# shaneson0/attacking_federate_learning

Measured on AMD Instinct MI355X. Metric: aggregation rounds/sec at N clients x D params (Bulyan), higher is better.
Workload: dtype f32 (Gram: fp16x2 split of every fp32 operand, 3 fp16 MFMAs per block, fp32/fp64 accumulate; <= 2e-7 of |gi||gj| vs f...

## Files before the change

attacking_federate_learning_amd/csrc/gram_planes.hip:

```cpp
#include "common.hpp"

#include <cstring>
#include <type_traits>

namespace byz {
namespace {

constexpr int kWgRows = 256;
constexpr int kWgCols = 128;
constexpr int kSlab = 128;
constexpr int kThreads = 512;
constexpr int kFragBytes = 1024;
constexpr int kRowBlocks = (kWgRows + kWgCols) / 32;
constexpr int kChunkCols = 8192;
constexpr int kChunkSteps = kChunkCols / 16;
constexpr int kFlushSteps = 16;
constexpr int kSpareRoundsPercent = 10;

typedef float f32x16 __attribute__((ext_vector_type(16)));
typedef float f32x4 __attribute__((ext_vector_type(4)));
typedef __bf16 bf16x8 __attribute__((ext_vector_type(8)));
typedef _Float16 f16x8 __attribute__((ext_vector_type(8)));
typedef uint32_t u32x4 __attribute__((ext_vector_type(4)));

// ... 590 lines not shown

    const int tid = threadIdx.x;
    const int lane = tid & 63;
    const int wave = __builtin_amdgcn_readfirstlane(tid >> 6);
    const unsigned where = static_cast<unsigned>(__builtin_amdgcn_readfirstlane(my_unit->wave[wave].where));
    const int a_slot = static_cast<int>(where & 0xffu);
    const int b_slot = static_cast<int>((where >> 8) & 0xffu);
    unsigned live_blocks = (where >> 16) & 0xffu;
    const int row_in_slab = static_cast<int>((where >> 24) & 1u) * 64;
    const int col_in_slab = static_cast<int>((where >> 25) & 1u) * 64;
    const int sum_slot = __builtin_amdgcn_readfirstlane(my_unit->wave[wave].sum_slot);
    const bool live_wave = live_blocks != 0;

    const int step0 = chunk * kChunkSteps;
    int n_stages = static_cast<int>(n_steps) - step0;
    if (n_stages > kChunkSteps) n_stages = kChunkSteps;
    const int n_super = n_stages / 2;

    int64_t piece_off[kPerWave];
#pragma unroll
    for (int i = 0; i < kPerWave; ++i) {
        const int q = wave + NW * i;
        const int rbl = q / PLANES, piece = q % PLANES;
        const int64_t rb = __builtin_amdgcn_readfirstlane(my_unit->rb[rbl]);
        piece_off[i] = (((rb * n_steps + step0) * PLANES + piece) * 64) * 16;
    }
    const unsigned char* lane_base = reinterpret_cast<const unsigned char*>(planes) + lane * 16;
    auto dma_piece = [&](int s, int i) __attribute__((always_inline)) {
        unsigned char* dst = lds + (s % NBUF) * kStage + wave * kFragBytes;
        __builtin_amdgcn_global_load_lds(
            (const __attribute__((address_space(1))) void*)(lane_base + piece_off[i] + static_cast<int64_t>(s) * (PLANES * kFragBytes)),
            (__attribute__((address_space(3))) void*)(dst + i * NW * kFragBytes), 16, 0, 0);
    };
    auto dma = [&](int s) __attribute__((always_inline)) {
#pragma unroll
        for (int i = 0; i < kPerWave; ++i) dma_piece(s, i);
    };

    f32x4 acc[4][4], acc2[4][4];
#pragma unroll
    for (int m = 0; m < 4; ++m)
#pragma unroll
        for (int n = 0; n < 4; ++n)
#pragma unroll
            for (int e = 0; e < 4; ++e) {
                acc[m][n][e] = 0.0f;
                acc2[m][n][e] = 0.0f;
            }

    const int lane_in_image = (lane & 15) + 32 * ((lane >> 4) & 1);
    const int pair_half = lane >> 5;
    auto frag_at = [&](int sp, int rb32, int h, int p) __attribute__((always_inline)) -> frag_t {
        const unsigned char* at = lds + (2 * (sp % (NBUF / 2)) + pair_half) * kStage + rb32 * kRbBytes + p * kFragBytes +
                                  (lane_in_image + 16 * h) * 16;
        return *reinterpret_cast<const frag_t*>(at);
    };
    struct AFrags { frag_t v[2][4]; };
    struct BFrags { frag_t v[2][2]; };
    auto read_a = [&](int sp, AFrags& a, auto mask_c) __attribute__((always_inline)) {
        constexpr unsigned MASK = decltype(mask_c)::value;
#pragma unroll
        for (int p = 0; p < 2; ++p)
#pragma unroll
            for (int m = 0; m < 4; ++m)
                if (((MASK >> ((m / 2) * 2)) & 3u) != 0) a.v[p][m] = frag_at(sp, a_slot + m / 2, m % 2, p);
    };
    auto read_b = [&](int sp, int half, BFrags& b, auto mask_c) __attribute__((always_inline)) {
        constexpr unsigned MASK = decltype(mask_c)::value;
#pragma unroll
        for (int p = 0; p < 2; ++p)
#pragma unroll
            for (int n = 0; n < 2; ++n) b.v[p][n] = frag_at(sp, b_slot + half, n, p);
        (void)MASK;
    };
    auto multiply_half = [&](const AFrags& a, const BFrags& b, auto half_c, auto mask_c) __attribute__((always_inline)) {
        constexpr unsigned MASK = decltype(mask_c)::value;
        constexpr int HALF = decltype(half_c)::value;
        constexpr int pa[3] = {1, 0, 0};
        constexpr int pb[3] = {0, 1, 0};
#pragma unroll
        for (int t = 0; t < 3; ++t)
#pragma unroll
            for (int m = 0; m < 4; ++m)
#pragma unroll
                for (int n = 0; n < 2; ++n)
                    if (((MASK >> ((m / 2) * 2 + HALF)) & 1u) != 0)
                        acc[m][2 * HALF + n] = __builtin_amdgcn_mfma_f32_16x16x32_f16(a.v[pa[t]][m], b.v[pb[t]][n], acc[m][2 * HALF + n], 0, 0, 0);
    };
    auto flush = [&](int sp) __attribute__((always_inline)) {
        if ((sp + 1) % kSuperFlush == 0) {
#pragma unroll
            for (int m = 0; m < 4; ++m)
#pragma unroll
                for (int n = 0; n < 4; ++n)
#pragma unroll
                    for (int e = 0; e < 4; ++e) {
                        acc2[m][n][e] += acc[m][n][e];
                        acc[m][n][e] = 0.0f;
                    }
        }
    };

    for (int a = 0; a < NBUF && a < n_stages; ++a) dma(a);
    {
        const int issued = n_stages < NBUF ? n_stages : NBUF;
        wait_vmcnt_dyn((issued > 2 ? issued - 2 : 0) * kPerWave);
    }
    asm volatile("s_barrier" ::: "memory");
    auto k_loop = [&](auto mask_c) __attribute__((always_inline)) {
        constexpr unsigned MASK = decltype(mask_c)::value;
        constexpr bool kLive = MASK != 0;
        constexpr std::integral_constant<int, 0> h0{};
        constexpr std::integral_constant<int, 1> h1{};
        AFrags a0, a1;
        BFrags b0, b1;
        if (kLive && n_super > 0) {
            read_a(0, a0, mask_c);
            if ((MASK & 5u) != 0) read_b(0, 0, b0, mask_c);
        }
        auto super = [&](int sp, AFrags& a, AFrags& an) __attribute__((always_inline)) {
            if (kLive) {
                if ((MASK & 10u) != 0) read_b(sp, 1, b1, mask_c);
                if ((MASK & 5u) != 0) multiply_half(a, b0, h0, mask_c);
            }
            {
                const int last = 2 * sp + 5 < n_stages - 1 ? 2 * sp + 5 : n_stages - 1;
                const int ahead = last - (2 * sp + 3);
                if (2 * sp + 7 < n_stages) wait_vmcnt<2 * kPerWave>();
                else wait_vmcnt_dyn((ahead > 0 ? ahead : 0) * kPerWave);
            }
            asm volatile("s_waitcnt lgkmcnt(0)\n\ts_barrier" ::: "memory");
            if (2 * sp + NBUF < n_stages) dma(2 * sp + NBUF);
            if (2 * sp + NBUF + 1 < n_stages) dma(2 * sp + NBUF + 1);
            if (kLive) {
                if (sp + 1 < n_super) {
                    read_a(sp + 1, an, mask_c);
                    if ((MASK & 5u) != 0) read_b(sp + 1, 0, b0, mask_c);
                }
                if ((MASK & 10u) != 0) multiply_half(a, b1, h1, mask_c);
                flush(sp);
            }
        };
        auto super8 = [&](int sp, AFrags& a, AFrags& an, auto pos_c) __attribute__((always_inline)) {
            constexpr int POS = decltype(pos_c)::value;
            constexpr bool FRESH = POS == 0, FLUSHING = POS == 7;
            constexpr int pa[3] = {1, 0, 0};
            constexpr int pb[3] = {0, 1, 0};
            const f32x4 zero4 = {0.0f, 0.0f, 0.0f, 0.0f};
            auto walk_n = [](int k) __attribute__((always_inline)) { return ((k / 2) & 1) ? 1 - k % 2 : k % 2; };
#pragma unroll
            for (int k = 0; k < 8; ++k) {
                const int m = k / 2, n = walk_n(k);
                if (k % 2 == 0) b1.v[k / 4][m % 2] = frag_at(sp, b_slot + 1, m % 2, k / 4);
#pragma unroll
                for (int t = 0; t < 3; ++t) {
                    acc[m][n] = __builtin_amdgcn_mfma_f32_16x16x32_f16(a.v[pa[t]][m], b0.v[pb[t]][n], (FRESH && t == 0) ? zero4 : acc[m][n], 0, 0, 0);
                    __builtin_amdgcn_sched_barrier(0);
                }
            }
            wait_vmcnt<2 * kPerWave>();
            asm volatile("s_waitcnt lgkmcnt(0)\n\ts_barrier" ::: "memory");
#pragma unroll
            for (int k = 0; k < 8; ++k) {
                const int m = k / 2, n = walk_n(k);
                if (k < 6) {
                    dma_piece(2 * sp + NBUF + k / 3, k % 3);
#pragma unroll
                    for (int r = 2 * k; r < 2 * k + 2; ++r) {
                        if (r < 8) an.v[r / 4][r % 4] = frag_at(sp + 1, a_slot + (r % 4) / 2, (r % 4) % 2, r / 4);
                        else b0.v[(r - 8) / 2][(r - 8) % 2] = frag_at(sp + 1, b_slot, (r - 8) % 2, (r - 8) / 2);
                    }
                }
#pragma unroll
                for (int t = 0; t < 3; ++t) {
                    acc[m][2 + n] = __builtin_amdgcn_mfma_f32_16x16x32_f16(a.v[pa[t]][m], b1.v[pb[t]][n], (FRESH && t == 0) ? zero4 : acc[m][2 + n], 0, 0, 0);
                    __builtin_amdgcn_sched_barrier(0);
                }
                if constexpr (FLUSHING) {
#pragma unroll
                    for (int e = 0; e < 4; ++e) acc2[m][k % 2][e] += acc[m][k % 2][e];
                }
            }
            if constexpr (FLUSHING) {
#pragma unroll
                for (int m = 0; m < 4; ++m)
#pragma unroll
                    for (int n = 2; n < 4; ++n)
#pragma unroll
                        for (int e = 0; e < 4; ++e) acc2[m][n][e] += acc[m][n][e];
            }
        };
        int sp = 0;
        if constexpr (MASK == 15u) {
            bool any = false;
            for (; 2 * (sp + 7) + NBUF + 1 < n_stages && sp + 8 < n_super; sp += 8) {
                super8(sp + 0, a0, a1, std::integral_constant<int, 0>{});
                super8(sp + 1, a1, a0, std::integral_constant<int, 1>{});
                super8(sp + 2, a0, a1, std::integral_constant<int, 2>{});
                super8(sp + 3, a1, a0, std::integral_constant<int, 3>{});
                super8(sp + 4, a0, a1, std::integral_constant<int, 4>{});
                super8(sp + 5, a1, a0, std::integral_constant<int, 5>{});
                super8(sp + 6, a0, a1, std::integral_constant<int, 6>{});
                super8(sp + 7, a1, a0, std::integral_constant<int, 7>{});
                any = true;
            }
            if (any) {
#pragma unroll
                for (int m = 0; m < 4; ++m)
#pragma unroll
                    for (int n = 0; n < 4; ++n)
#pragma unroll
                        for (int e = 0; e < 4; ++e) acc[m][n][e] = 0.0f;
            }
        }
        for (; sp + 1 < n_super; sp += 2) {
            super(sp, a0, a1);
            super(sp + 1, a1, a0);
        }
        if (sp < n_super) super(sp, a0, a1);
    };
    switch (live_blocks) {
        case 0u: k_loop(std::integral_constant<unsigned, 0u>{}); break;
        case 1u: k_loop(std::integral_constant<unsigned, 1u>{}); break;
        case 3u: k_loop(std::integral_constant<unsigned, 3u>{}); break;
        case 13u: k_loop(std::integral_constant<unsigned, 13u>{}); break;
        default: live_blocks = 15u; k_loop(std::integral_constant<unsigned, 15u>{}); break;
    }
    auto block_live = [&](int m, int n) __attribute__((always_inline)) { return ((live_blocks >> ((m / 2) * 2 + n / 2)) & 1u) != 0; };

    if constexpr (DEFER) {
        if (live_wave) {
            const bool unflushed = (n_super % kSuperFlush) != 0;
            float* out = chunk_sums + (static_cast<int64_t>(chunk) * n_sum_slots + sum_slot) * (kSlab * kSlab);
            float* rag = ragged_sums + static_cast<int64_t>(sum_slot) * (kSlab * kSlab);
#pragma unroll
            for (int m = 0; m < 4; ++m)
#pragma unroll
                for (int n = 0; n < 4; ++n) {
                    if (!block_live(m, n)) continue;
                    const int j = col_in_slab + 16 * n + (lane & 15);
#pragma unroll
                    for (int e = 0; e < 4; ++e) {
                        const int i = row_in_slab + 16 * m + 4 * (lane >> 4) + e;
                        out[i * kSlab + j] = acc2[m][n][e];
                        if (unflushed) rag[i * kSlab + j] = acc[m][n][e];
                    }
                }
        }
        __syncthreads();
        if (tid == 0) __hip_atomic_fetch_add(done, 1, __ATOMIC_RELAXED, __HIP_MEMORY_SCOPE_AGENT);
        return;
    }
    bool lost = false;
    if (chunk > 0) {
        if (tid == 0) {
            unsigned spins = 0;
            while (__hip_atomic_load(tickets + t_list, __ATOMIC_RELAXED, __HIP_MEMORY_SCOPE_AGENT) != chunk) {
                __builtin_amdgcn_s_sleep(8);
                if (++spins > (1u << 26)) {
                    lost = true;
                    break;
                }
            }
            __builtin_amdgcn_fence(__ATOMIC_ACQUIRE, "agent");
        }
        lost = __syncthreads_or(lost ? 1 : 0) != 0;
    }
    if (lost) {
        if (tid == 0) atomicOr(device_status, kStatusLostTicket);
    } else if (live_wave) {
        const bool slab_live = chunk > 0 || slab_live0 != 0;
        const int slab = __builtin_amdgcn_readfirstlane(my_unit->wave[wave].slab);
        const int ti = slab & 0xffff, tj = slab >> 16;
        double* out = partial + (static_cast<int64_t>(ti) * (ti + 1) / 2 + tj) * (kSlab * kSlab);
        const double* un = unscale + static_cast<int64_t>(chunk) * rows_pad;
#pragma unroll
        for (int m = 0; m < 4; ++m)
#pragma unroll
            for (int n = 0; n < 4; ++n) {
                if (!block_live(m, n)) continue;
                const int j = col_in_slab + 16 * n + (lane & 15);
                const double uj = un[static_cast<int64_t>(tj) * kSlab + j];
#pragma unroll
                for (int e = 0; e < 4; ++e) {
                    const int i = row_in_slab + 16 * m + 4 * (lane >> 4) + e;
                    double v = static_cast<double>(acc2[m][n][e]);
                    v += static_cast<double>(acc[m][n][e]);
                    v *= un[static_cast<int64_t>(ti) * kSlab + i] * uj;
                    if (slab_live) v += out[i * kSlab + j];
                    out[i * kSlab + j] = v;
                }
            }
    }
    asm volatile("s_waitcnt vmcnt(0)" ::: "memory");
    __syncthreads();
    if (tid == 0) {
        __builtin_amdgcn_fence(__ATOMIC_RELEASE, "agent");
        asm volatile("s_waitcnt vmcnt(0)" ::: "memory");
        __hip_atomic_store(tickets + t_list, chunk + 1, __ATOMIC_RELAXED, __HIP_MEMORY_SCOPE_AGENT);
        __hip_atomic_fetch_add(done, 1, __ATOMIC_RELAXED, __HIP_MEMORY_SCOPE_AGENT);
    }
}

constexpr int kReduceRun = 8;
__global__ __launch_bounds__(256) void chunk_reduce_kernel(const float* __restrict__ chunk_sums, const float* __restrict__ ragged_sums,
                                                           int n_sum_slots, int n_chunks, int ragged_chunk,
                                                           const int2* __restrict__ slot_slab, const double* __restrict__ unscale,
                                                           int64_t rows_pad, double* __restrict__ partial, int slab_live0,
                                                           int n_blocks32) {
    typedef double f64x4 __attribute__((ext_vector_type(4)));
    const int slot = blockIdx.x;
    const int2 tt = slot_slab[slot];
    const int ti = tt.x, tj = tt.y;
    if (ti < 0) return;
    double* out = partial + (static_cast<int64_t>(ti) * (ti + 1) / 2 + tj) * (kSlab * kSlab);
    const int64_t slab_stride = static_cast<int64_t>(n_sum_slots) * (kSlab * kSlab);
    const float* in = chunk_sums + static_cast<int64_t>(slot) * (kSlab * kSlab);
    const float* rag = ragged_sums + static_cast<int64_t>(slot) * (kSlab * kSlab);
    const int i = static_cast<int>(blockIdx.y) * 32 + (threadIdx.x >> 3), j = (threadIdx.x & 7) * 4;
    for (int jb = 0; jb < kSlab; jb += 32) {
        const int jj = jb + j;
        if (n_blocks32 >= 0) {
            const int rblk = ti * 4 + (i >> 5), cblk = tj * 4 + (jj >> 5);
            if (!(rblk < n_blocks32 && cblk <= rblk)) continue;
        }
        const int idx = i * kSlab + jj;
        f64x4 v = {0.0, 0.0, 0.0, 0.0};
        bool live = slab_live0 != 0;
        if (live) v = *reinterpret_cast<const f64x4*>(out + idx);
        for (int c0 = 0; c0 < n_chunks; c0 += kReduceRun) {
            f32x4 p[kReduceRun];
            double ui[kReduceRun];
            f64x4 uj[kReduceRun];
#pragma unroll
            for (int k = 0; k < kReduceRun; ++k) {
                const int c = c0 + k < n_chunks ? c0 + k : n_chunks - 1;
                p[k] = *reinterpret_cast<const f32x4*>(in + c * slab_stride + idx);
                const double* un = unscale + static_cast<int64_t>(c) * rows_pad;
                ui[k] = un[static_cast<int64_t>(ti) * kSlab + i];
                uj[k] = *reinterpret_cast<const f64x4*>(un + static_cast<int64_t>(tj) * kSlab + jj);
            }
#pragma unroll
            for (int k = 0; k < kReduceRun; ++k) {
                if (c0 + k >= n_chunks) break;
                f64x4 q = {static_cast<double>(p[k][0]), static_cast<double>(p[k][1]), static_cast<double>(p[k][2]),
                           static_cast<double>(p[k][3])};
                if (c0 + k == ragged_chunk) {
                    const f32x4 r = *reinterpret_cast<const f32x4*>(rag + idx);
                    q[0] += static_cast<double>(r[0]); q[1] += static_cast<double>(r[1]);
                    q[2] += static_cast<double>(r[2]); q[3] += static_cast<double>(r[3]);
                }
#pragma unroll
                for (int e = 0; e < 4; ++e) {
                    q[e] *= ui[k] * uj[k][e];
                    v[e] = live ? q[e] + v[e] : q[e];
                }
                live = true;
            }
        }
        *reinterpret_cast<f64x4*>(out + idx) = v;
    }
}

}

bool gram_planes_enabled() { return env_int("BYZ_GRAM_PLANES", 1) != 0; }

void build_gram_units(int64_t t128, int64_t n_blocks32, bool diagonal_units, int share_count, int share_index,
                      std::vector<GramUnit>& units, std::vector<int32_t>& slot_slab) {
    units.clear();
    slot_slab.clear();
    const int64_t t256 = ceil_div(t128, 2);
    auto live_mask = [&](int64_t ti, int64_t tj, int row64, int col64) -> uint32_t {
        if (!(tj <= ti && ti < t128)) return 0u;
        if (n_blocks32 < 0) return 15u;
        uint32_t mask = 0;
        for (int m = 0; m < 2; ++m)
            for (int n = 0; n < 2; ++n) {
                const int64_t rblk = ti * 4 + row64 * 2 + m, cblk = tj * 4 + col64 * 2 + n;
                if (rblk < n_blocks32 && cblk <= rblk) mask |= 1u << (m * 2 + n);
            }
        return mask;
    };
    auto set_wave = [&](GramUnit& u, int wave, int a_slot, int b_slot, int64_t ti, int64_t tj, int row64, int col64,
                        int64_t sum_slot) {
        const uint32_t mask = live_mask(ti, tj, row64, col64);
        GramUnitWave& w = u.wave[wave];
        w.where = static_cast<uint32_t>(a_slot) | static_cast<uint32_t>(b_slot) << 8 | mask << 16 |
                  static_cast<uint32_t>(row64) << 24 | static_cast<uint32_t>(col64) << 25;
        w.sum_slot = mask != 0 ? static_cast<int32_t>(sum_slot) : 0;
        w.slab = mask != 0 ? static_cast<int32_t>(ti | tj << 16) : 0;
    };
    auto slab_slot = [](int64_t ti, int64_t tj) { return ti * (ti + 1) / 2 + tj; };
    int64_t position = 0;
    auto plain = [&](int64_t bi, int64_t tj, bool d1) {
        if (position++ % share_count != share_index) return;
        const int64_t t_list = static_cast<int64_t>(units.size());
        GramUnit u{};
        for (int s = 0; s < 12; ++s) u.rb[s] = static_cast<int32_t>(s < 8 ? bi * 8 + s : tj * 4 + (s - 8));
        for (int wave = 0; wave < 8; ++wave) {
            const int wr = wave / 2, wc = wave % 2;
            const int64_t ti = 2 * bi + wr / 2;
            set_wave(u, wave, 2 * wr, 8 + 2 * wc, ti, tj, wr % 2, wc, diagonal_units ? slab_slot(ti, tj) : 2 * t_list + wr / 2);
        }
        if (d1) set_wave(u, 1, 4, 4, 2 * bi + 1, 2 * bi + 1, 0, 0, slab_slot(2 * bi + 1, 2 * bi + 1));
        units.push_back(u);
        if (!diagonal_units)
            for (int sel = 0; sel < 2; ++sel) {
                const int64_t ti = 2 * bi + sel;
                const bool live = tj <= ti && ti < t128;
                slot_slab.push_back(static_cast<int32_t>(live ? ti : -1));
                slot_slab.push_back(static_cast<int32_t>(live ? tj : -1));
            }
    };
    auto d2 = [&](int64_t first, int64_t count) {
        static const int partial_wave[3] = {3, 7, 5};
        GramUnit u{};
        for (int s = 0; s < 12; ++s) u.rb[s] = static_cast<int32_t>(first * 8 + 4);
        for (int64_t k = 0; k < count; ++k) {
            const int64_t bi = first + k, t = 2 * bi + 1;
            for (int s = 0; s < 4; ++s) u.rb[4 * k + s] = static_cast<int32_t>(bi * 8 + 4 + s);
            set_wave(u, static_cast<int>(k), static_cast<int>(4 * k + 2), static_cast<int>(4 * k), t, t, 1, 0, slab_slot(t, t));
            set_wave(u, partial_wave[k], static_cast<int>(4 * k + 2), static_cast<int>(4 * k + 2), t, t, 1, 1, slab_slot(t, t));
        }
        units.push_back(u);
    };
    const int64_t full_blocks = t128 / 2;
    for (int64_t b0 = 0; b0 < t256; b0 += 4)
        for (int64_t tj = 0; tj < t128 && tj <= 2 * (b0 + 3) + 1; ++tj)
            for (int64_t bi = b0; bi < b0 + 4 && bi < t256; ++bi) {
                if (tj > 2 * bi + 1) continue;
                if (!diagonal_units) {
                    plain(bi, tj, false);
                } else if (tj == 2 * bi + 1) {
                    if (bi % 3 == 2 || bi == full_blocks - 1) d2(bi - bi % 3, bi % 3 + 1);
                } else {
                    plain(bi, tj, tj == 2 * bi);
                }
            }
    if (diagonal_units)
        for (int64_t ti = 0; ti < t128; ++ti)
            for (int64_t tj = 0; tj <= ti; ++tj) {
                slot_slab.push_back(static_cast<int32_t>(ti));
                slot_slab.push_back(static_cast<int32_t>(tj));
            }
}

int launch_gram_planes(byz_ctx* ctx, const float* G, int64_t n_rows, int64_t n_cols, int64_t ld, const int32_t* row_index,
                       double* slabs, int share_count, int share_index, uint8_t* owned_host, bool f16, hipStream_t stream) {
    const int64_t t128 = ceil_div(n_rows, kSlab);
    const int64_t t256 = ceil_div(t128, 2);
    const int64_t rows_pad = t256 * kWgRows;
    bool defer = f16 && env_int("BYZ_GRAM_DEFER", 1) != 0;
    const int n_blocks32 = env_int("BYZ_GRAM_BLOCK_SKIP", 1) != 0 ? static_cast<int>(ceil_div(n_rows, 32)) : -1;
    auto ensure_list = [&](bool diagonal_units) -> int {
        const int64_t order_key = static_cast<int64_t>((f16 ? 1 : 0) + (diagonal_units ? 2 : 0)) * (1ll << 40) + share_count * 65536 + share_index;
        const int64_t blocks_key = f16 ? n_blocks32 : -2;
        if (ctx->plane_order_T != t128 || ctx->plane_order_share != order_key || ctx->plane_order_blocks != blocks_key) {
            ctx->plane_order_host.clear();
            if (f16) {
                if (t128 > 0x7fff) {
                    set_error("gram: more than 32767 slabs per side");
                    return BYZ_E_UNSUPPORTED;
                }
                std::vector<GramUnit> units;
                std::vector<int32_t> slot_slab;
                build_gram_units(t128, n_blocks32, diagonal_units, share_count, share_index, units, slot_slab);
                ctx->plane_units = static_cast<int64_t>(units.size());
                ctx->plane_sum_slots = static_cast<int64_t>(slot_slab.size() / 2);
                ctx->plane_order_host.resize(units.size() * kGramUnitWords);
                if (!units.empty()) std::memcpy(ctx->plane_order_host.data(), units.data(), units.size() * sizeof(GramUnit));
                ctx->plane_order_host.insert(ctx->plane_order_host.end(), slot_slab.begin(), slot_slab.end());
            } else {
                int64_t position = 0;
                auto push = [&](int64_t bi, int64_t tj) {
                    if (position++ % share_count != share_index) return;
                    ctx->plane_order_host.push_back(static_cast<int32_t>(bi));
                    ctx->plane_order_host.push_back(static_cast<int32_t>(tj));
                };
                const int64_t S = ceil_div(t128, 8);
                for (int64_t I = 0; I < S; ++I)
                    for (int64_t J = 0; J <= I; ++J)
                        for (int64_t bi = I * 4; bi < I * 4 + 4 && bi < t256; ++bi)
                            for (int64_t tj = J * 8; tj < J * 8 + 8 && tj <= 2 * bi + 1 && tj < t128; ++tj) push(bi, tj);
                ctx->plane_units = static_cast<int64_t>(ctx->plane_order_host.size() / 2);
                ctx->plane_sum_slots = 0;
            }
            BYZ_TRY(ctx->plane_order.ensure(ctx->plane_order_host.size() * sizeof(int32_t) + 16));
            BYZ_HIP(hipMemcpyAsync(ctx->plane_order.ptr, ctx->plane_order_host.data(),
                                   ctx->plane_order_host.size() * sizeof(int32_t), hipMemcpyHostToDevice, stream));
            BYZ_HIP(hipStreamSynchronize(stream));
            ctx->plane_order_T = t128;
            ctx->plane_order_share = order_key;
            ctx->plane_order_blocks = blocks_key;
        }
        return BYZ_OK;
    };
    const bool diagonal_units = defer && share_count == 1 && n_blocks32 >= 0;
    BYZ_TRY(ensure_list(diagonal_units));
    int64_t n_tiles = ctx->plane_units;
    int64_t n_sum_slots = ctx->plane_sum_slots;
    const int32_t* slot_slab_host = ctx->plane_order_host.data() + n_tiles * kGramUnitWords;
    if (owned_host != nullptr) {
        if (f16) {
            for (int64_t s = 0; s < n_sum_slots; ++s) {
                const int64_t ti = slot_slab_host[2 * s], tj = slot_slab_host[2 * s + 1];
                if (ti >= 0) owned_host[ti * (ti + 1) / 2 + tj] = 1;
            }
        } else {
            for (int64_t t = 0; t < n_tiles; ++t) {
                const int64_t bi = ctx->plane_order_host[2 * t], tj = ctx->plane_order_host[2 * t + 1];
                for (int64_t ti = 2 * bi; ti < 2 * bi + 2 && ti < t128; ++ti)
                    if (tj <= ti) owned_host[ti * (ti + 1) / 2 + tj] = 1;
            }
        }
    }
    if (n_tiles == 0) return BYZ_OK;

    const int n_planes = f16 ? 2 : 3;
    size_t free_b = 0, total_b = 0;
    BYZ_HIP(hipMemGetInfo(&free_b, &total_b));
    int64_t budget = static_cast<int64_t>(env_int("BYZ_GRAM_PLANE_MB", 16384)) << 20;
    const int64_t have = static_cast<int64_t>(ctx->gram_planes.bytes);
    if (budget > have + static_cast<int64_t>(free_b / 2)) budget = have + static_cast<int64_t>(free_b / 2);
    int64_t chunks_per_sc = budget / (rows_pad * 2 * n_planes * kChunkCols);
    const int64_t chunks_total = ceil_div(n_cols, kChunkCols);
    if (chunks_per_sc > chunks_total) chunks_per_sc = chunks_total;
    if (chunks_per_sc < 1) {
        set_error("gram: no room for one 8192-column chunk of 16-bit planes (%lld rows)", (long long)rows_pad);
        return BYZ_E_HIP;
    }
    const int64_t n_sc = ceil_div(chunks_total, chunks_per_sc);
    chunks_per_sc = ceil_div(chunks_total, n_sc);
    const int64_t sc_cols = chunks_per_sc * kChunkCols;
    BYZ_TRY(ctx->gram_planes.ensure(static_cast<size_t>(rows_pad) * 2 * n_planes * sc_cols));
    double* unscale = nullptr;
    if (f16) {
        BYZ_TRY(ctx->plane_unscale.ensure(static_cast<size_t>(rows_pad) * chunks_per_sc * sizeof(double)));
        unscale = ctx->plane_unscale.as<double>();
    }
    u32x4* planes = ctx->gram_planes.as<u32x4>();
    float* chunk_sums = nullptr;
    float* ragged_sums = nullptr;
    if (defer) {
        const size_t per_chunk = static_cast<size_t>(n_sum_slots) * kSlab * kSlab * sizeof(float);
        const size_t want = per_chunk * static_cast<size_t>(chunks_per_sc + 1);
        size_t free_now = 0, total_now = 0;
        BYZ_HIP(hipMemGetInfo(&free_now, &total_now));
        if (want > ctx->gram_chunk_sums.bytes && want - ctx->gram_chunk_sums.bytes > free_now / 2) defer = false;
        if (!defer && diagonal_units) {
            BYZ_TRY(ensure_list(false));
            n_tiles = ctx->plane_units;
            n_sum_slots = ctx->plane_sum_slots;
        }
    }
    if (defer) {
        const size_t per_chunk = static_cast<size_t>(n_sum_slots) * kSlab * kSlab * sizeof(float);
        BYZ_TRY(ctx->gram_chunk_sums.ensure(per_chunk * static_cast<size_t>(chunks_per_sc + 1)));
        chunk_sums = ctx->gram_chunk_sums.as<float>();
        ragged_sums = chunk_sums + (per_chunk / sizeof(float)) * static_cast<size_t>(chunks_per_sc);
    }
    auto kernel16 = defer ? &gram_planes16_kernel<6, true> : &gram_planes16_kernel<6, false>;
    const void* kernel = f16 ? reinterpret_cast<const void*>(kernel16) : reinterpret_cast<const void*>(&gram_planes_kernel<4>);
    const size_t lds_bytes = static_cast<size_t>(f16 ? 6 : 4) * kRowBlocks * n_planes * kFragBytes;
    BYZ_HIP(allow_dynamic_lds(ctx, kernel, static_cast<int>(lds_bytes)));
    const int round_size = env_int("BYZ_GRAM_ROUND", ctx->num_cus / 8);
    const int run = round_size > 0 ? round_size : ctx->num_cus / 8;
    const int64_t per_xcd = ceil_div(n_tiles, 8);
    for (int64_t sc = 0; sc < n_sc; ++sc) {
        const int64_t k0 = sc * sc_cols;
        const int64_t cols = n_cols - k0 < sc_cols ? n_cols - k0 : sc_cols;
        const int64_t n_steps = ceil_div(cols, 32) * 2;
        const int64_t n_chunks = ceil_div(n_steps, kChunkSteps);
        {
            KernelTimer t(ctx, BYZ_K_PLANE_SPLIT, stream);
            if (f16) {
                const dim3 grid(static_cast<unsigned>(n_chunks), static_cast<unsigned>(rows_pad / 32));
                if (env_int("BYZ_GRAM_SPLIT_TWO_PASS", 0) != 0) {
                    plane_split_f16_kernel<<<grid, 256, 0, stream>>>(G, n_rows, n_cols, ld, row_index, k0, n_steps, planes,
                                                                     unscale, rows_pad, nullptr);
                } else {
                    const int64_t pairs = n_chunks * (rows_pad / 32);
                    BYZ_TRY(ctx->split_redo.ensure(static_cast<size_t>(1 + 2 * pairs) * sizeof(int32_t)));
                    int32_t* redo = ctx->split_redo.as<int32_t>();
                    BYZ_HIP(hipMemsetAsync(redo, 0, sizeof(int32_t), stream));
                    plane_split_f16_stream_kernel<<<grid, 256, 0, stream>>>(G, n_rows, n_cols, ld, row_index, k0, n_steps, planes,
                                                                            unscale, rows_pad, redo);
                    BYZ_TRY(check_launch("plane_split_f16_stream_kernel"));
                    const int64_t fix = pairs < 4096 ? pairs : 4096;
                    plane_split_f16_kernel<<<static_cast<unsigned>(fix), 256, 0, stream>>>(G, n_rows, n_cols, ld, row_index, k0,
                                                                                           n_steps, planes, unscale, rows_pad, redo);
                }
            } else {
                const dim3 grid(static_cast<unsigned>(ceil_div(n_steps, kSplitCols / 16)), static_cast<unsigned>(rows_pad / 32));
                plane_split_bf16_kernel<<<grid, 256, 0, stream>>>(G, n_rows, n_cols, ld, row_index, k0, n_steps, planes);
            }
            BYZ_TRY(check_launch("plane_split_kernel"));
        }
        {
            int64_t rounds_per_xcd = 0;
            if (f16) {
                rounds_per_xcd = ceil_div(ceil_div(n_tiles * n_chunks, run), 8);
                rounds_per_xcd += rounds_per_xcd * kSpareRoundsPercent / 100;
            }
            const int64_t grid = f16 ? 8 * run * rounds_per_xcd : 8 * per_xcd * n_chunks;
            const size_t ticket_ints = static_cast<size_t>(n_tiles + 9 + 8 * rounds_per_xcd);
            BYZ_TRY(ctx->gram_tickets.ensure(ticket_ints * sizeof(int)));
            int* tickets = ctx->gram_tickets.as<int>();
            BYZ_HIP(hipMemsetAsync(tickets, 0, ticket_ints * sizeof(int), stream));
            KernelTimer t(ctx, BYZ_K_GRAM, stream);
            if (grid > 0x7fffffff) {
                set_error("gram: grid too large");
                return BYZ_E_UNSUPPORTED;
            }
            const int slab_live0 = sc > 0 ? 1 : 0;
            if (!f16) {
                gram_planes_kernel<4><<<static_cast<unsigned>(grid), kThreads, lds_bytes, stream>>>(
                    planes, n_steps, slabs, static_cast<int>(n_tiles), ctx->plane_order.as<int2>(), static_cast<int>(n_chunks), tickets,
                    round_size, static_cast<int>(t128), slab_live0, n_blocks32, device_status_word(ctx));
            } else {
                kernel16<<<static_cast<unsigned>(grid), kThreads, lds_bytes, stream>>>(
                    planes, n_steps, unscale, rows_pad, slabs, static_cast<int>(n_tiles), ctx->plane_order.as<GramUnit>(),
                    static_cast<int>(n_chunks), tickets, round_size, run, slab_live0, static_cast<int>(n_sum_slots),
                    device_status_word(ctx), chunk_sums, ragged_sums);
            }
            BYZ_TRY(check_launch("gram_planes_kernel"));
        }
        if (defer) {
            KernelTimer t(ctx, BYZ_K_GRAM_REDUCE, stream);
            const int ragged_chunk = (n_steps % kChunkSteps) % kFlushSteps != 0 ? static_cast<int>(n_chunks) - 1 : -1;
            const int2* slot_slab = reinterpret_cast<const int2*>(ctx->plane_order.as<GramUnit>() + n_tiles);
            chunk_reduce_kernel<<<dim3(static_cast<unsigned>(n_sum_slots), 4), 256, 0, stream>>>(
                chunk_sums, ragged_sums, static_cast<int>(n_sum_slots), static_cast<int>(n_chunks), ragged_chunk, slot_slab,
                unscale, rows_pad, slabs, sc > 0 ? 1 : 0, n_blocks32);
            BYZ_TRY(check_launch("chunk_reduce_kernel"));
        }
    }
    return BYZ_OK;
}

}
```

Baseline: 2.058.

## Skip dead row blocks in plane split and retile chunk reduction

The chunk reduction kernel is remapped so each block covers 16 rows by 128 columns, two rows per thread. Whole blocks now exit early when their 32-row block is dead, instead of looping over column groups. Gram units redirect row-block slots no wave reads to slot 0, so those planes are not loaded. The plane split grid shrinks to the highest row block any unit references, and the unscale buffer is zeroed on growth so unsplit rows hold defined values. This cuts wasted split work and memory traffic, at the cost of more host-side scanning and a more complex slot mapping.

```diff
diff --git a/attacking_federate_learning_amd/csrc/gram_planes.hip b/attacking_federate_learning_amd/csrc/gram_planes.hip
--- a/attacking_federate_learning_amd/csrc/gram_planes.hip
+++ b/attacking_federate_learning_amd/csrc/gram_planes.hip
@@ -917,6 +917,7 @@
 }
 
 constexpr int kReduceRun = 8;
+constexpr int kReduceRows = 16;
 __global__ __launch_bounds__(256) void chunk_reduce_kernel(const float* __restrict__ chunk_sums, const float* __restrict__ ragged_sums,
                                                            int n_sum_slots, int n_chunks, int ragged_chunk,
                                                            const int2* __restrict__ slot_slab, const double* __restrict__ unscale,
@@ -927,53 +928,61 @@
     const int2 tt = slot_slab[slot];
     const int ti = tt.x, tj = tt.y;
     if (ti < 0) return;
+    const int i = static_cast<int>(blockIdx.y) * kReduceRows + (threadIdx.x >> 5), j = (threadIdx.x & 31) * 4;
+    if (n_blocks32 >= 0) {
+        const int rblk = ti * 4 + (i >> 5), cblk = tj * 4 + (j >> 5);
+        if (!(rblk < n_blocks32 && cblk <= rblk)) return;
+    }
     double* out = partial + (static_cast<int64_t>(ti) * (ti + 1) / 2 + tj) * (kSlab * kSlab);
     const int64_t slab_stride = static_cast<int64_t>(n_sum_slots) * (kSlab * kSlab);
     const float* in = chunk_sums + static_cast<int64_t>(slot) * (kSlab * kSlab);
     const float* rag = ragged_sums + static_cast<int64_t>(slot) * (kSlab * kSlab);
-    const int i = static_cast<int>(blockIdx.y) * 32 + (threadIdx.x >> 3), j = (threadIdx.x & 7) * 4;
-    for (int jb = 0; jb < kSlab; jb += 32) {
-        const int jj = jb + j;
-        if (n_blocks32 >= 0) {
-            const int rblk = ti * 4 + (i >> 5), cblk = tj * 4 + (jj >> 5);
-            if (!(rblk < n_blocks32 && cblk <= rblk)) continue;
-        }
-        const int idx = i * kSlab + jj;
-        f64x4 v = {0.0, 0.0, 0.0, 0.0};
-        bool live = slab_live0 != 0;
-        if (live) v = *reinterpret_cast<const f64x4*>(out + idx);
-        for (int c0 = 0; c0 < n_chunks; c0 += kReduceRun) {
-            f32x4 p[kReduceRun];
-            double ui[kReduceRun];
-            f64x4 uj[kReduceRun];
-#pragma unroll
-            for (int k = 0; k < kReduceRun; ++k) {
-                const int c = c0 + k < n_chunks ? c0 + k : n_chunks - 1;
-                p[k] = *reinterpret_cast<const f32x4*>(in + c * slab_stride + idx);
-                const double* un = unscale + static_cast<int64_t>(c) * rows_pad;
-                ui[k] = un[static_cast<int64_t>(ti) * kSlab + i];
-                uj[k] = *reinterpret_cast<const f64x4*>(un + static_cast<int64_t>(tj) * kSlab + jj);
-            }
-#pragma unroll
-            for (int k = 0; k < kReduceRun; ++k) {
-                if (c0 + k >= n_chunks) break;
-                f64x4 q = {static_cast<double>(p[k][0]), static_cast<double>(p[k][1]), static_cast<double>(p[k][2]),
-                           static_cast<double>(p[k][3])};
+    const int idx[2] = {i * kSlab + j, (i + 8) * kSlab + j};
+    const double* un_i = unscale + static_cast<int64_t>(ti) * kSlab + i;
+    const double* un_j = unscale + static_cast<int64_t>(tj) * kSlab + j;
+    f64x4 v[2] = {{0.0, 0.0, 0.0, 0.0}, {0.0, 0.0, 0.0, 0.0}};
+    bool live = slab_live0 != 0;
+    if (live) {
+#pragma unroll
+        for (int r = 0; r < 2; ++r) v[r] = *reinterpret_cast<const f64x4*>(out + idx[r]);
+    }
+    for (int c0 = 0; c0 < n_chunks; c0 += kReduceRun) {
+        f32x4 p[kReduceRun][2];
+        double ui[kReduceRun][2];
+        f64x4 uj[kReduceRun];
+#pragma unroll
+        for (int k = 0; k < kReduceRun; ++k) {
+            const int c = c0 + k < n_chunks ? c0 + k : n_chunks - 1;
+#pragma unroll
+            for (int r = 0; r < 2; ++r) {
+                p[k][r] = *reinterpret_cast<const f32x4*>(in + c * slab_stride + idx[r]);
+                ui[k][r] = un_i[static_cast<int64_t>(c) * rows_pad + 8 * r];
+            }
+            uj[k] = *reinterpret_cast<const f64x4*>(un_j + static_cast<int64_t>(c) * rows_pad);
+        }
+#pragma unroll
+        for (int k = 0; k < kReduceRun; ++k) {
+            if (c0 + k >= n_chunks) break;
+#pragma unroll
+            for (int r = 0; r < 2; ++r) {
+                f64x4 q = {static_cast<double>(p[k][r][0]), static_cast<double>(p[k][r][1]), static_cast<double>(p[k][r][2]),
+                           static_cast<double>(p[k][r][3])};
                 if (c0 + k == ragged_chunk) {
-                    const f32x4 r = *reinterpret_cast<const f32x4*>(rag + idx);
-                    q[0] += static_cast<double>(r[0]); q[1] += static_cast<double>(r[1]);
-                    q[2] += static_cast<double>(r[2]); q[3] += static_cast<double>(r[3]);
+                    const f32x4 t = *reinterpret_cast<const f32x4*>(rag + idx[r]);
+                    q[0] += static_cast<double>(t[0]); q[1] += static_cast<double>(t[1]);
+                    q[2] += static_cast<double>(t[2]); q[3] += static_cast<double>(t[3]);
                 }
 #pragma unroll
                 for (int e = 0; e < 4; ++e) {
-                    q[e] *= ui[k] * uj[k][e];
-                    v[e] = live ? q[e] + v[e] : q[e];
-                }
-                live = true;
-            }
-        }
-        *reinterpret_cast<f64x4*>(out + idx) = v;
-    }
+                    q[e] *= ui[k][r] * uj[k][e];
+                    v[r][e] = live ? q[e] + v[r][e] : q[e];
+                }
+            }
+            live = true;
+        }
+    }
+#pragma unroll
+    for (int r = 0; r < 2; ++r) *reinterpret_cast<f64x4*>(out + idx[r]) = v[r];
 }
 
 }
@@ -1006,18 +1015,33 @@
         w.slab = mask != 0 ? static_cast<int32_t>(ti | tj << 16) : 0;
     };
     auto slab_slot = [](int64_t ti, int64_t tj) { return ti * (ti + 1) / 2 + tj; };
+    auto retire_dead_slots = [](GramUnit& u) {
+        uint32_t read = 0;
+        for (int wave = 0; wave < 8; ++wave) {
+            const uint32_t where = u.wave[wave].where;
+            const uint32_t a_slot = where & 0xffu, b_slot = (where >> 8) & 0xffu, mask = (where >> 16) & 0xffu;
+            for (int k = 0; k < 2; ++k) {
+                if (((mask >> (2 * k)) & 3u) != 0) read |= 1u << (a_slot + k);
+                if (((mask >> k) & 5u) != 0) read |= 1u << (b_slot + k);
+            }
+        }
+        for (int s = 1; s < 12; ++s)
+            if (((read >> s) & 1u) == 0) u.rb[s] = u.rb[0];
+    };
     int64_t position = 0;
     auto plain = [&](int64_t bi, int64_t tj, bool d1) {
         if (position++ % share_count != share_index) return;
         const int64_t t_list = static_cast<int64_t>(units.size());
         GramUnit u{};
         for (int s = 0; s < 12; ++s) u.rb[s] = static_cast<int32_t>(s < 8 ? bi * 8 + s : tj * 4 + (s - 8));
+        const int b_base = tj == 2 * bi ? 0 : tj == 2 * bi + 1 ? 4 : 8;
         for (int wave = 0; wave < 8; ++wave) {
             const int wr = wave / 2, wc = wave % 2;
             const int64_t ti = 2 * bi + wr / 2;
-            set_wave(u, wave, 2 * wr, 8 + 2 * wc, ti, tj, wr % 2, wc, diagonal_units ? slab_slot(ti, tj) : 2 * t_list + wr / 2);
+            set_wave(u, wave, 2 * wr, b_base + 2 * wc, ti, tj, wr % 2, wc, diagonal_units ? slab_slot(ti, tj) : 2 * t_list + wr / 2);
         }
         if (d1) set_wave(u, 1, 4, 4, 2 * bi + 1, 2 * bi + 1, 0, 0, slab_slot(2 * bi + 1, 2 * bi + 1));
+        retire_dead_slots(u);
         units.push_back(u);
         if (!diagonal_units)
             for (int sel = 0; sel < 2; ++sel) {
@@ -1037,6 +1061,7 @@
             set_wave(u, static_cast<int>(k), static_cast<int>(4 * k + 2), static_cast<int>(4 * k), t, t, 1, 0, slab_slot(t, t));
             set_wave(u, partial_wave[k], static_cast<int>(4 * k + 2), static_cast<int>(4 * k + 2), t, t, 1, 1, slab_slot(t, t));
         }
+        retire_dead_slots(u);
         units.push_back(u);
     };
     const int64_t full_blocks = t128 / 2;
@@ -1150,7 +1175,9 @@
     BYZ_TRY(ctx->gram_planes.ensure(static_cast<size_t>(rows_pad) * 2 * n_planes * sc_cols));
     double* unscale = nullptr;
     if (f16) {
+        const size_t before = ctx->plane_unscale.bytes;
         BYZ_TRY(ctx->plane_unscale.ensure(static_cast<size_t>(rows_pad) * chunks_per_sc * sizeof(double)));
+        if (ctx->plane_unscale.bytes != before) BYZ_HIP(hipMemsetAsync(ctx->plane_unscale.ptr, 0, ctx->plane_unscale.bytes, stream));
         unscale = ctx->plane_unscale.as<double>();
     }
     u32x4* planes = ctx->gram_planes.as<u32x4>();
@@ -1173,6 +1200,15 @@
         BYZ_TRY(ctx->gram_chunk_sums.ensure(per_chunk * static_cast<size_t>(chunks_per_sc + 1)));
         chunk_sums = ctx->gram_chunk_sums.as<float>();
         ragged_sums = chunk_sums + (per_chunk / sizeof(float)) * static_cast<size_t>(chunks_per_sc);
+    }
+    int64_t split_blocks = rows_pad / 32;
+    if (f16) {
+        split_blocks = 0;
+        for (int64_t t = 0; t < n_tiles; ++t)
+            for (int s = 0; s < kRowBlocks; ++s) {
+                const int64_t rb = ctx->plane_order_host[t * kGramUnitWords + s];
+                if (rb + 1 > split_blocks) split_blocks = rb + 1;
+            }
     }
     auto kernel16 = defer ? &gram_planes16_kernel<6, true> : &gram_planes16_kernel<6, false>;
     const void* kernel = f16 ? reinterpret_cast<const void*>(kernel16) : reinterpret_cast<const void*>(&gram_planes_kernel<4>);
@@ -1189,12 +1225,12 @@
         {
             KernelTimer t(ctx, BYZ_K_PLANE_SPLIT, stream);
             if (f16) {
-                const dim3 grid(static_cast<unsigned>(n_chunks), static_cast<unsigned>(rows_pad / 32));
+                const dim3 grid(static_cast<unsigned>(n_chunks), static_cast<unsigned>(split_blocks));
                 if (env_int("BYZ_GRAM_SPLIT_TWO_PASS", 0) != 0) {
                     plane_split_f16_kernel<<<grid, 256, 0, stream>>>(G, n_rows, n_cols, ld, row_index, k0, n_steps, planes,
                                                                      unscale, rows_pad, nullptr);
                 } else {
-                    const int64_t pairs = n_chunks * (rows_pad / 32);
+                    const int64_t pairs = n_chunks * split_blocks;
                     BYZ_TRY(ctx->split_redo.ensure(static_cast<size_t>(1 + 2 * pairs) * sizeof(int32_t)));
                     int32_t* redo = ctx->split_redo.as<int32_t>();
                     BYZ_HIP(hipMemsetAsync(redo, 0, sizeof(int32_t), stream));
@@ -1244,7 +1280,7 @@
             KernelTimer t(ctx, BYZ_K_GRAM_REDUCE, stream);
             const int ragged_chunk = (n_steps % kChunkSteps) % kFlushSteps != 0 ? static_cast<int>(n_chunks) - 1 : -1;
             const int2* slot_slab = reinterpret_cast<const int2*>(ctx->plane_order.as<GramUnit>() + n_tiles);
-            chunk_reduce_kernel<<<dim3(static_cast<unsigned>(n_sum_slots), 4), 256, 0, stream>>>(
+            chunk_reduce_kernel<<<dim3(static_cast<unsigned>(n_sum_slots), kSlab / kReduceRows), 256, 0, stream>>>(
                 chunk_sums, ragged_sums, static_cast<int>(n_sum_slots), static_cast<int>(n_chunks), ragged_chunk, slot_slab,
                 unscale, rows_pad, slabs, sc > 0 ? 1 : 0, n_blocks32);
             BYZ_TRY(check_launch("chunk_reduce_kernel"));
```

Result: no change. 2.068, median of 6 (+0.5%).

## Restructure chunk reduce with LDS-staged unscale factors and skip padded split rows

Applied to the files above, without the earlier changes.

Rewrites chunk_reduce_kernel so each block handles an 8-row strip with 32 threads spanning a full row. Per-chunk row and column unscale factors are staged once in shared memory instead of each thread loading them, chunk sums use nontemporal loads, and blocks whose rows fall outside the valid 32-row blocks exit early. The split kernel launches only over real rows when deferring diagonal units, and newly allocated plane and unscale buffers are zeroed so the skipped padded rows stay well defined. This adds barriers per chunk group and extra memsets on reallocation.

```diff
diff --git a/attacking_federate_learning_amd/csrc/gram_planes.hip b/attacking_federate_learning_amd/csrc/gram_planes.hip
--- a/attacking_federate_learning_amd/csrc/gram_planes.hip
+++ b/attacking_federate_learning_amd/csrc/gram_planes.hip
@@ -916,64 +916,74 @@
     }
 }
 
-constexpr int kReduceRun = 8;
+constexpr int kReduceRun = 4;
+constexpr int kReduceRows = 8;
 __global__ __launch_bounds__(256) void chunk_reduce_kernel(const float* __restrict__ chunk_sums, const float* __restrict__ ragged_sums,
                                                            int n_sum_slots, int n_chunks, int ragged_chunk,
                                                            const int2* __restrict__ slot_slab, const double* __restrict__ unscale,
                                                            int64_t rows_pad, double* __restrict__ partial, int slab_live0,
                                                            int n_blocks32) {
     typedef double f64x4 __attribute__((ext_vector_type(4)));
-    const int slot = blockIdx.x;
+    __shared__ __attribute__((aligned(32))) double u_col[kReduceRun][kSlab];
+    __shared__ double u_row[kReduceRun][kReduceRows];
+    const int slot = static_cast<int>(blockIdx.x) / (kSlab / kReduceRows);
+    const int strip = static_cast<int>(blockIdx.x) % (kSlab / kReduceRows);
     const int2 tt = slot_slab[slot];
     const int ti = tt.x, tj = tt.y;
     if (ti < 0) return;
-    double* out = partial + (static_cast<int64_t>(ti) * (ti + 1) / 2 + tj) * (kSlab * kSlab);
+    const int tid = threadIdx.x;
+    const int ri = tid >> 5, i = strip * kReduceRows + ri, jj = (tid & 31) * 4;
+    const int rblk = ti * 4 + (i >> 5), cblk = tj * 4 + (jj >> 5);
+    if (n_blocks32 >= 0 && rblk >= n_blocks32) return;
+    const bool mine = n_blocks32 < 0 || cblk <= rblk;
+    const int idx = i * kSlab + jj;
+    double* out = partial + (static_cast<int64_t>(ti) * (ti + 1) / 2 + tj) * (kSlab * kSlab) + idx;
     const int64_t slab_stride = static_cast<int64_t>(n_sum_slots) * (kSlab * kSlab);
-    const float* in = chunk_sums + static_cast<int64_t>(slot) * (kSlab * kSlab);
-    const float* rag = ragged_sums + static_cast<int64_t>(slot) * (kSlab * kSlab);
-    const int i = static_cast<int>(blockIdx.y) * 32 + (threadIdx.x >> 3), j = (threadIdx.x & 7) * 4;
-    for (int jb = 0; jb < kSlab; jb += 32) {
-        const int jj = jb + j;
-        if (n_blocks32 >= 0) {
-            const int rblk = ti * 4 + (i >> 5), cblk = tj * 4 + (jj >> 5);
-            if (!(rblk < n_blocks32 && cblk <= rblk)) continue;
-        }
-        const int idx = i * kSlab + jj;
-        f64x4 v = {0.0, 0.0, 0.0, 0.0};
-        bool live = slab_live0 != 0;
-        if (live) v = *reinterpret_cast<const f64x4*>(out + idx);
-        for (int c0 = 0; c0 < n_chunks; c0 += kReduceRun) {
-            f32x4 p[kReduceRun];
-            double ui[kReduceRun];
-            f64x4 uj[kReduceRun];
+    const float* in = chunk_sums + static_cast<int64_t>(slot) * (kSlab * kSlab) + idx;
+    const float* rag = ragged_sums + static_cast<int64_t>(slot) * (kSlab * kSlab) + idx;
+    f64x4 v = {0.0, 0.0, 0.0, 0.0};
+    bool live = slab_live0 != 0;
+    if (live && mine) v = *reinterpret_cast<const f64x4*>(out);
+    for (int c0 = 0; c0 < n_chunks; c0 += kReduceRun) {
+        f32x4 p[kReduceRun];
+        if (mine) {
 #pragma unroll
             for (int k = 0; k < kReduceRun; ++k) {
                 const int c = c0 + k < n_chunks ? c0 + k : n_chunks - 1;
-                p[k] = *reinterpret_cast<const f32x4*>(in + c * slab_stride + idx);
-                const double* un = unscale + static_cast<int64_t>(c) * rows_pad;
-                ui[k] = un[static_cast<int64_t>(ti) * kSlab + i];
-                uj[k] = *reinterpret_cast<const f64x4*>(un + static_cast<int64_t>(tj) * kSlab + jj);
-            }
-#pragma unroll
-            for (int k = 0; k < kReduceRun; ++k) {
-                if (c0 + k >= n_chunks) break;
-                f64x4 q = {static_cast<double>(p[k][0]), static_cast<double>(p[k][1]), static_cast<double>(p[k][2]),
-                           static_cast<double>(p[k][3])};
-                if (c0 + k == ragged_chunk) {
-                    const f32x4 r = *reinterpret_cast<const f32x4*>(rag + idx);
-                    q[0] += static_cast<double>(r[0]); q[1] += static_cast<double>(r[1]);
-                    q[2] += static_cast<double>(r[2]); q[3] += static_cast<double>(r[3]);
-                }
-#pragma unroll
-                for (int e = 0; e < 4; ++e) {
-                    q[e] *= ui[k] * uj[k][e];
-                    v[e] = live ? q[e] + v[e] : q[e];
-                }
-                live = true;
-            }
-        }
-        *reinterpret_cast<f64x4*>(out + idx) = v;
-    }
+                p[k] = __builtin_nontemporal_load(reinterpret_cast<const f32x4*>(in + c * slab_stride));
+            }
+        }
+        __syncthreads();
+        for (int e = tid; e < kReduceRun * (kSlab + kReduceRows); e += 256) {
+            const int k = e / (kSlab + kReduceRows), w = e % (kSlab + kReduceRows);
+            const int c = c0 + k < n_chunks ? c0 + k : n_chunks - 1;
+            const double* un = unscale + static_cast<int64_t>(c) * rows_pad;
+            if (w < kSlab) u_col[k][w] = un[static_cast<int64_t>(tj) * kSlab + w];
+            else u_row[k][w - kSlab] = un[static_cast<int64_t>(ti) * kSlab + strip * kReduceRows + (w - kSlab)];
+        }
+        __syncthreads();
+        if (!mine) continue;
+#pragma unroll
+        for (int k = 0; k < kReduceRun; ++k) {
+            if (c0 + k >= n_chunks) break;
+            f64x4 q = {static_cast<double>(p[k][0]), static_cast<double>(p[k][1]), static_cast<double>(p[k][2]),
+                       static_cast<double>(p[k][3])};
+            if (c0 + k == ragged_chunk) {
+                const f32x4 r = *reinterpret_cast<const f32x4*>(rag);
+                q[0] += static_cast<double>(r[0]); q[1] += static_cast<double>(r[1]);
+                q[2] += static_cast<double>(r[2]); q[3] += static_cast<double>(r[3]);
+            }
+            const double ui = u_row[k][ri];
+            const f64x4 uj = *reinterpret_cast<const f64x4*>(&u_col[k][jj]);
+#pragma unroll
+            for (int e = 0; e < 4; ++e) {
+                q[e] *= ui * uj[e];
+                v[e] = live ? q[e] + v[e] : q[e];
+            }
+            live = true;
+        }
+    }
+    if (mine) *reinterpret_cast<f64x4*>(out) = v;
 }
 
 }
@@ -1148,9 +1158,14 @@
     chunks_per_sc = ceil_div(chunks_total, n_sc);
     const int64_t sc_cols = chunks_per_sc * kChunkCols;
     BYZ_TRY(ctx->gram_planes.ensure(static_cast<size_t>(rows_pad) * 2 * n_planes * sc_cols));
+    if (static_cast<int64_t>(ctx->gram_planes.bytes) != have)
+        BYZ_HIP(hipMemsetAsync(ctx->gram_planes.ptr, 0, ctx->gram_planes.bytes, stream));
     double* unscale = nullptr;
     if (f16) {
+        const size_t had = ctx->plane_unscale.bytes;
         BYZ_TRY(ctx->plane_unscale.ensure(static_cast<size_t>(rows_pad) * chunks_per_sc * sizeof(double)));
+        if (ctx->plane_unscale.bytes != had)
+            BYZ_HIP(hipMemsetAsync(ctx->plane_unscale.ptr, 0, ctx->plane_unscale.bytes, stream));
         unscale = ctx->plane_unscale.as<double>();
     }
     u32x4* planes = ctx->gram_planes.as<u32x4>();
@@ -1189,12 +1204,13 @@
         {
             KernelTimer t(ctx, BYZ_K_PLANE_SPLIT, stream);
             if (f16) {
-                const dim3 grid(static_cast<unsigned>(n_chunks), static_cast<unsigned>(rows_pad / 32));
+                const int64_t split_blocks = defer && diagonal_units ? ceil_div(n_rows, 32) : rows_pad / 32;
+                const dim3 grid(static_cast<unsigned>(n_chunks), static_cast<unsigned>(split_blocks));
                 if (env_int("BYZ_GRAM_SPLIT_TWO_PASS", 0) != 0) {
                     plane_split_f16_kernel<<<grid, 256, 0, stream>>>(G, n_rows, n_cols, ld, row_index, k0, n_steps, planes,
                                                                      unscale, rows_pad, nullptr);
                 } else {
-                    const int64_t pairs = n_chunks * (rows_pad / 32);
+                    const int64_t pairs = n_chunks * split_blocks;
                     BYZ_TRY(ctx->split_redo.ensure(static_cast<size_t>(1 + 2 * pairs) * sizeof(int32_t)));
                     int32_t* redo = ctx->split_redo.as<int32_t>();
                     BYZ_HIP(hipMemsetAsync(redo, 0, sizeof(int32_t), stream));
@@ -1244,7 +1260,11 @@
             KernelTimer t(ctx, BYZ_K_GRAM_REDUCE, stream);
             const int ragged_chunk = (n_steps % kChunkSteps) % kFlushSteps != 0 ? static_cast<int>(n_chunks) - 1 : -1;
             const int2* slot_slab = reinterpret_cast<const int2*>(ctx->plane_order.as<GramUnit>() + n_tiles);
-            chunk_reduce_kernel<<<dim3(static_cast<unsigned>(n_sum_slots), 4), 256, 0, stream>>>(
+            if (n_sum_slots * (kSlab / kReduceRows) > 0x7fffffff) {
+                set_error("gram: grid too large");
+                return BYZ_E_UNSUPPORTED;
+            }
+            chunk_reduce_kernel<<<static_cast<unsigned>(n_sum_slots * (kSlab / kReduceRows)), 256, 0, stream>>>(
                 chunk_sums, ragged_sums, static_cast<int>(n_sum_slots), static_cast<int>(n_chunks), ragged_chunk, slot_slab,
                 unscale, rows_pad, slabs, sc > 0 ? 1 : 0, n_blocks32);
             BYZ_TRY(check_launch("chunk_reduce_kernel"));
```

Result: no change. 2.100 before, 2.111 after, median of 5 (+0.5%).
